# Orca0917/TransformerTTS

Hardware: AMD Instinct MI355X
Metric: mel frames/sec teacher-forced step, LJSpeech-shape batch, 1/2/4/8 MI355X (higher is better)
Workload: dtype f32; 1 GPU; BASELINE configs[2] (batch 64, 1 GPU; per-GPU shard of configs[3]): training step (no-grad fwd + fwd + loss + bwd + clip + Adam), batch 64/GPU x 870 frames x 100 phonemes (dense), base config d_model 256, 3+3 layers, dropout on, fp32; global_batch=64, parallelism=dp1, batch_stream=one resident batch, accumulate=1, process_group=none, grad_allreduce=none (1 GPU), alignments_written=True, dma_gemms=True, layernorm_images=False, head_images=True, fused_cross_kv=True, wgrad_groups=True, twin_encoder=True, twin_postnet=True

## Files before the change

include/ttts_hip.h:

```cpp
#ifndef TTTS_HIP_H
#define TTTS_HIP_H

#include <stddef.h>
#include <stdint.h>

#ifdef __cplusplus
extern "C" {
#endif

#define TTTS_OK 0
#define TTTS_ERR_INVALID (-1)
#define TTTS_ERR_LAUNCH (-2)

#define TTTS_AMAX_SLOTS 1024

#define TTTS_ACT_NONE 0
#define TTTS_ACT_RELU 1
#define TTTS_ACT_TANH 2

typedef struct ttts_step_state {
    uint64_t seed;
    float lr;
    float p_tf;
    int64_t step;
// ... 261 lines not shown
                      const int64_t* frames, const uint8_t* mask, int64_t ld_mask, int B, int Tmax, int Pmax, float* mean,
                      int32_t* counts, void* stream);
int ttts_length_regulate_frames(void);
int ttts_length_regulate_fwd(const float* x, int64_t ld_row, int64_t ld_batch, const int64_t* durations, const int64_t* phoneme_lens,
                             int B, int Pmax, int Tmax, int D, float* y, int64_t* mel_lens, int32_t* index, void* stream);
int ttts_length_regulate_bwd(const float* dy, const int64_t* durations, const int64_t* phoneme_lens, int B, int Pmax, int Tmax, int D,
                             float* dx, int accumulate, void* stream);
int ttts_durations_from_log(const float* log_d, const int64_t* phoneme_lens, int B, int Pmax, float alpha, int64_t min_duration,
                            int64_t* durations, void* stream);
int ttts_variance_embed_fwd(const float* x, int64_t ld_row, int64_t ld_batch, const float* pitch, const float* energy,
                            const float* pitch_bins, int n_pitch, const float* energy_bins, int n_energy, const float* pitch_table,
                            const float* energy_table, const int64_t* phoneme_lens, int B, int Pmax, int D, float* y,
                            int64_t* pitch_ids, int64_t* energy_ids, void* stream);
int ttts_variance_loss_fwd(const float* log_d_pred, const int64_t* durations, const float* pitch_pred, const float* pitch_target,
                           const float* energy_pred, const float* energy_target, const int64_t* phoneme_lens, int B, int Pmax, float w_d,
                           float w_p, float w_e, float* out, void* stream);
int ttts_variance_loss_bwd(const float* log_d_pred, const int64_t* durations, const float* pitch_pred, const float* pitch_target,
                           const float* energy_pred, const float* energy_target, const int64_t* phoneme_lens, int B, int Pmax, float w_d,
                           float w_p, float w_e, const float* gout, float* d_log_d, float* d_pitch, float* d_energy, void* stream);
int ttts_heads_pad_w(const float* src, int64_t ld_src, float* dst, int64_t rows, int H, int head_dim, int width, void* stream);
int ttts_heads_unpad_w(const float* src, float* dst, int64_t ld_dst, int64_t rows, int H, int head_dim, int width, void* stream);
int ttts_attention_fwd_img(const void* q, const void* k, const void* v, const float* q_inv, const float* k_inv,
                           const float* v_inv, float* o, float* lse, float* attn, const int64_t* key_lens, int B, int H, int Tq,
                           int Tk, int ldq, int ldk, int ldv, int ldo, int causal, float q_scale, float drop_p, uint64_t seed,
                           const uint64_t* step_seed, const float* v_amax, float* o_amax_out, float* rowstat_out, int64_t q_inv_rows, int64_t k_inv_rows, int64_t stat_plane,
                           void* stream);
int ttts_attention_bwd_img(const void* q, const void* k, const void* v, const float* q_inv, const float* k_inv,
                           const float* v_inv, const float* o, const float* d_o, const float* rowstat, float* delta, float* dq,
                           float* dk, float* dv, const int64_t* key_lens, int B, int H, int Tq, int Tk, int ldq, int ldk, int ldv,
                           int ldo, int lddq, int lddk, int lddv, int causal, float q_scale, float drop_p, uint64_t seed,
                           const uint64_t* step_seed, const float* do_amax, float* dq_amax_out, float* dkv_amax_out,
                           float* dkv_partials , int q_splits ,
                           int64_t q_inv_rows, int64_t k_inv_rows, int64_t stat_plane, void* stream);

int ttts_embedding_fwd(const int64_t* ids, const float* table, float* out, int64_t n, int vocab, int d,
                       float* out_amax_out , void* stream);
int ttts_embedding_bwd(const int64_t* ids, const float* dout, float* dtable, int64_t n, int vocab, int d, int accumulate,
                       void* stream);
int ttts_posenc_fwd(const float* x, const float* pe, const float* alpha, float* y, int B, int T, int d, float drop_p,
                    uint64_t seed, const uint64_t* step_seed, float* y_amax_out , void* stream);
size_t ttts_posenc_bwd_workspace_bytes(void);
int ttts_posenc_bwd(const float* dy, const float* pe, float* dx, float* dalpha, float* ws, size_t ws_bytes, int B, int T,
                    int d, float drop_p, uint64_t seed, const uint64_t* step_seed, int accumulate, void* stream);
int ttts_relu_dropout_bwd(const float* dy, const float* out, float* dx, int64_t n, float drop_p, float* dx_amax_out,
                          void* stream);
int ttts_dropout_bwd(const float* dy, float* dx, int64_t n, float drop_p, uint64_t seed, const uint64_t* step_seed,
                     float* dx_amax_out, void* stream);
int ttts_zero(void* p, size_t nbytes, void* stream);
int ttts_add(const float* x, const float* y, float* z, int64_t n, void* stream);
int ttts_add3(const float* x, const float* y, const float* w, float* z, int64_t n, void* stream);
int ttts_collate_melspec(const float* ragged, const int64_t* frame_offsets, float* out, int B, int Tmax, int n_mels,
                         void* stream);
int ttts_collate_phoneme(const int64_t* ragged, const int64_t* offsets, int64_t* out, int B, int Pmax, void* stream);

int ttts_rowdot_fwd(const float* x, const float* w, const float* b, float* y, int64_t M, int d, void* stream);
size_t ttts_rowdot_bwd_workspace_bytes(int d);
int ttts_rowdot_bwd(const float* dy, const float* x, const float* w, float* dx_accum, float* dw, float* db, float* ws,
                    size_t ws_bytes, int64_t M, int d, int accumulate, ttts_reduce_queue* queue, void* stream);

size_t ttts_loss_workspace_bytes(void);
int ttts_loss_fwd(const float* pred, const float* post, const float* stop, const float* mel, const int64_t* lens,
                  float* out4, float* ws, size_t ws_bytes, int B, int T, int C, float pos_weight, void* stream);
int ttts_loss_bwd(const float* pred, const float* post, const float* stop, const float* mel, const int64_t* lens,
                  const float* ws, const float* g_total, const float* g_pred_mel, const float* g_post_mel, const float* g_stop,
                  float* dpred, float* dpost, float* dstop, int B, int T, int C, float pos_weight, void* stream);
int ttts_sched_sampling_mix(const float* pred, const float* mel, const float* u, const int64_t* lens, float* out, int B,
// ... 53 lines not shown
```

transformertts_amd/_lib.py:

```python
from __future__ import annotations

import ctypes
import os
from ctypes import c_char_p, c_float, c_int, c_int64, c_size_t, c_uint64, c_void_p

import torch

_HERE = os.path.dirname(os.path.abspath(__file__))
LIB_PATH = os.environ.get("TTTS_LIB", os.path.join(_HERE, "libttts_hip.so"))

P, I, L, F, U, Z = c_void_p, c_int, c_int64, c_float, c_uint64, c_size_t

SIGNATURES = {
    "ttts_last_error": (c_char_p, []),
    "ttts_abi_version": (I, []),
    "ttts_linear_fwd": (I, [P, P, P, P, P, L, I, I, I, F, U, P, I, I, P]),
    "ttts_linear_bwd_data": (I, [P, P, P, P, L, I, I, P, F, P]),
    "ttts_wgrad_workspace_bytes": (Z, [L, I, I, I]),
    "ttts_linear_bwd_weight": (I, [P, P, P, P, P, Z, L, I, I, I, I, I, P, P]),
    "ttts_split_bytes": (Z, [L, L]),
    "ttts_split_image_bytes": (Z, [L, L, I, I, I]),
    "ttts_gemm_tile_choice": (I, [L, I, I, I]),
    "ttts_weight_split": (I, [P, P, I, I, I, I, I, P]),
    "ttts_weight_split_units": (L, [L, L, I, I]),
# ... 19 lines not shown
    "ttts_linear_bwd_data_x6": (I, [P, P, P, P, L, I, I, P, F, P]),
    "ttts_conv1d_fwd_x6": (I, [P, P, P, P, I, I, I, I, I, P]),
    "ttts_conv1d_bwd_data_x6": (I, [P, P, P, I, I, I, I, I, P]),
    "ttts_linear_bwd_weight_x6": (I, [P, P, P, P, P, Z, L, I, I, I, I, I, P, P]),
    "ttts_conv1d_bwd_weight_x6": (I, [P, P, P, P, P, Z, I, I, I, I, I, I, P, P]),
    "ttts_linear_bwd_weight_h3": (I, [P, P, P, P, P, Z, L, I, I, I, I, I, P, P, P, P]),
    "ttts_conv1d_bwd_weight_h3": (I, [P, P, P, P, P, Z, I, I, I, I, I, I, P, P, P, P]),
    "ttts_linear_bwd_weight_h3_parts": (I, [P, P, P, P, I, P, Z, L, I, I, I, P, P, P, P]),
    "ttts_wgrad_group_ok": (I, [L, I, I, I]),
    "ttts_wgrad_group": (I, [I, P, P, P, P, P, P, P, P, P, P, P, P, I, P, P, P, P]),
    "ttts_conv1d_pack_bytes": (Z, [I, I, I]),
    "ttts_conv1d_pack_weight": (I, [P, P, P, I, I, I, P]),
    "ttts_conv1d_fwd": (I, [P, P, P, P, I, I, I, I, I, P]),
    "ttts_conv1d_bwd_data": (I, [P, P, P, I, I, I, I, I, P]),
    "ttts_conv1d_bwd_weight": (I, [P, P, P, P, P, Z, I, I, I, I, I, I, P, P]),
    "ttts_bn_workspace_bytes": (Z, [L, I]),
    "ttts_bn_train_stats": (I, [P, P, P, P, P, P, P, Z, L, I, F, F, P]),
    "ttts_bn_eval_stats": (I, [P, P, P, P, I, F, P]),
    "ttts_bn_apply_fwd": (I, [P, P, P, P, P, P, L, I, I, F, U, P, P, P]),
    "ttts_bn_bwd": (I, [P, P, P, P, P, P, P, P, P, P, Z, L, I, I, F, U, P, I, P, I, P]),
    "ttts_layernorm_fwd": (I, [P, P, P, P, P, P, L, I, F, P, P, P, P]),
    "ttts_layernorm_bwd_workspace_bytes": (Z, [I]),
    "ttts_layernorm_bwd": (I, [P, P, P, P, P, P, P, P, P, Z, L, I, I, P, P, P, P]),
    "ttts_layernorm_bwd_drop": (I, [P, P, P, P, P, P, P, P, P, Z, L, I, I, P, F, U, P, P, P, P, P, P]),
    "ttts_attention_fwd": (I, [P, P, P, P, P, P, P, I, I, I, I, I, I, I, I, I, F, F, U, P, P]),
    "ttts_attention_fwd_x6": (I, [P, P, P, P, P, P, P, I, I, I, I, I, I, I, I, I, F, F, U, P, P]),
    "ttts_attention_fwd_h3": (I, [P, P, P, P, P, P, P, I, I, I, I, I, I, I, I, I, F, F, U, P, P, P, P, P, P, P]),
    "ttts_attention_bwd": (I, [P, P, P, P, P, P, P, P, P, P, P, I, I, I, I, I, I, I, I, I, I, I, I, F, F, U, P, P]),
    "ttts_attention_bwd_x6": (I, [P, P, P, P, P, P, P, P, P, P, P, I, I, I, I, I, I, I, I, I, I, I, I, F, F, U, P, P]),
    "ttts_attention_bwd_h3": (I, [P, P, P, P, P, P, P, P, P, P, P, I, I, I, I, I, I, I, I, I, I, I, I, F, F, U, P, P, P, P, P, P, P, P, P]),
    "ttts_attention_fwd_img": (I, [P, P, P, P, P, P, P, P, P, P, I, I, I, I, I, I, I, I, I, F, F, U, P, P, P, P, L, L, L, P]),
    "ttts_attention_bwd_img": (I, [P, P, P, P, P, P, P, P, P, P, P, P, P, P, I, I, I, I, I, I, I, I, I, I, I, I, F, F, U, P, P, P, P,
                                   P, I, L, L, L, P]),
    "ttts_attention_fwd_wide": (I, [P, P, P, P, P, P, P, I, I, I, I, I, I, I, I, I, F, F, U, P, P]),
    "ttts_attention_bwd_wide": (I, [P, P, P, P, P, P, P, P, P, P, P, I, I, I, I, I, I, I, I, I, I, I, I, F, F, U, P, P]),
    "ttts_attention_fwd_wide_masked": (I, [P, P, P, P, P, P, P, I, I, I, I, I, I, I, I, I, F, F, U, P, P, L, L, L, P, L, P]),
    "ttts_attention_bwd_wide_masked": (I, [P, P, P, P, P, P, P, P, P, P, P, I, I, I, I, I, I, I, I, I, I, I, I, F, F, U, P, P, L, L, L,
                                           P, L, P]),
    "ttts_attention_bwd_wide_dattn": (I, [P, P, P, P, P, P, P, P, P, P, P, I, I, I, I, I, I, I, I, I, I, I, I, F, F, U, P, P, L, L, L,
                                          P, L, P, P, L, L, L, P]),
    "ttts_guided_attention_fwd": (I, [P, P, P, U, F, I, I, I, I, P, I, I, I, P, P]),
    "ttts_guided_attention_bwd": (I, [P, P, P, U, F, I, I, I, I, I, I, P, P]),
    "ttts_alignment_rowstats": (I, [P, L, L, L, P, P, I, I, I, I, I, I, P, P, P, P]),
    "ttts_alignment_select": (I, [P, P, P, I, I, I, I, I, I, P, P, P]),
    "ttts_alignment_durations_argmax": (I, [P, P, P, P, I, I, I, I, I, P, P, P]),
    "ttts_alignment_mas_workspace_bytes": (Z, [I, I, I]),
    "ttts_alignment_mas": (I, [P, I, L, L, L, P, P, P, I, I, I, I, P, Z, P, P, P]),
    "ttts_dtw_workspace_bytes": (Z, [I, I, I]),
    "ttts_dtw": (I, [P, L, L, P, P, L, L, P, I, I, I, I, I, P, Z, P, P, P, P, P, P]),
    "ttts_audio_tables_bytes": (Z, [I, I, I]),
    "ttts_audio_tables_check": (I, [P, Z, I, I, I, I]),
    "ttts_logmel": (I, [P, L, P, I, I, I, I, I, I, P, F, P, P, P, I, P]),
    "ttts_logmel_stats": (I, [P, P, I, I, I, P, P]),
    "ttts_vocoder_pinv_check": (I, [P, Z, I, I]),
    "ttts_mel_to_magnitude": (I, [P, L, L, P, I, I, I, I, I, P, P, F, P, P, P]),
    "ttts_istft": (I, [P, P, I, I, I, I, P, P, P, P]),
    "ttts_stft_project": (I, [P, L, P, P, I, I, I, I, P, P, P, F, P, P, P]),
    "ttts_resample_table_bytes": (Z, [I, I]),
    "ttts_resample_table_check": (I, [P, Z, I, I, I]),
    "ttts_resample_tile": (I, []),
    "ttts_resample": (I, [P, L, P, I, I, I, I, I, P, P, L, P, P]),
    "ttts_pitch_lags": (I, []),
    "ttts_pitch_frames": (I, [I, I, I, I, I]),
    "ttts_pitch_block": (I, [I, I, I, I, I]),
    "ttts_pitch_energy": (I, [P, L, P, I, I, I, I, I, I, I, I, I, F, F, P, P, P, P, P, P, P]),
    "ttts_segment_mean": (I, [P, L, P, P, P, P, L, I, I, I, P, P, P]),
# ... 84 lines not shown
```

transformertts_amd/csrc/attention_img.hip:

```cpp
#include "attention_common.h"

namespace ttts {

struct AttnImgArgs {
    const void* q; const void* k; const void* v;
    const float* q_inv; const float* k_inv; const float* v_inv;
    long q_rows, k_rows;
    long stat_plane;
    float* o; float* lse; float* attn;
    const float* dout; float* delta; float* dq; float* dk; float* dv;
    const int64_t* key_lens;
    int B, H, Tq, Tk;
    int ldq, ldk, ldv, ldo, lddq, lddk, lddv;
    float qscale;
    float drop_scale; uint32_t thr; uint64_t seed; const uint64_t* step_seed;
    const float* v_amax;
    const float* do_amax;
    float* amax_dq; float* amax_dkv;
    float* dkv_part; long part_stride;
    int ldp;
    float* o_amax;
    float* rowstat;
};

// ... 1075 lines not shown
        const float fv = inv_g / H3A_P * a.drop_scale;
        float mx = 0.f;
#pragma unroll
        for (int r = 0; r < 16; ++r) {
            dk[0][r] *= fk; dk[1][r] *= fk; dv[0][r] *= fv; dv[1][r] *= fv;
            mx = fmaxf(fmaxf(mx, fmaxf(fabsf(dk[0][r]), fabsf(dk[1][r]))), fmaxf(fabsf(dv[0][r]), fabsf(dv[1][r])));
        }
        if (a.amax_dkv != nullptr && gridDim.z == 1) amax_publish(kg < a.Tk ? mx : 0.f, a.amax_dkv, blockIdx.y * gridDim.x + blockIdx.x);
    }
    if (gridDim.z == 1) {
        wave_store_rows4(dk, scratch4, a.dk + (long)b * a.Tk * a.lddk + h * HD, kw0, a.Tk, a.lddk, lane);
        wave_store_rows4(dv, scratch4, a.dv + (long)b * a.Tk * a.lddv + h * HD, kw0, a.Tk, a.lddv, lane);
    } else {
        float* part = a.dkv_part + (long)blockIdx.z * a.part_stride + (long)b * a.Tk * a.ldp + h * HD;
        wave_store_rows4(dk, scratch4, part, kw0, a.Tk, a.ldp, lane);
        wave_store_rows4(dv, scratch4, part + a.H * HD, kw0, a.Tk, a.ldp, lane);
    }
}

__global__ __launch_bounds__(256) void attn_dkv_reduce_kernel(const float* __restrict__ part, float* __restrict__ out, long n4, int zs,
                                                              long stride, float* __restrict__ amax, int cols4, long out_ld) {
    float mx = 0.f;
    for (long i = (long)blockIdx.x * blockDim.x + threadIdx.x; i < n4; i += (long)gridDim.x * blockDim.x) {
        float4 acc = reinterpret_cast<const float4*>(part)[i];
        for (int z = 1; z < zs; ++z) {
            const float4 v = reinterpret_cast<const float4*>(part + (long)z * stride)[i];
            acc.x += v.x; acc.y += v.y; acc.z += v.z; acc.w += v.w;
        }
        const long row = i / cols4;
        *reinterpret_cast<float4*>(out + row * out_ld + (i - row * cols4) * 4) = acc;
        mx = fmaxf(fmaxf(mx, fmaxf(fabsf(acc.x), fabsf(acc.y))), fmaxf(fabsf(acc.z), fabsf(acc.w)));
    }
    if (amax != nullptr) amax_publish(mx, amax, blockIdx.x * 4 + (threadIdx.x >> 6));
}

#ifndef TTTS_AIMG_KT
#define TTTS_AIMG_KT 32
#endif

static int check_img_spans(const char* name, int Tq, int Tk, int ldq, int ldk, int ldv) {
    TTTS_REQUIRE((uint64_t)Tq * ldq * 4 < (1ull << 32) && (uint64_t)Tk * ldk * 4 < (1ull << 32) && (uint64_t)Tk * ldv * 4 < (1ull << 32),
                 "%s: one utterance's operand exceeds 4 GiB", name);
    return TTTS_OK;
}
static int fill_img_planes(const char* name, AttnImgArgs& a, int B, int H, int Tq, int Tk, int64_t q_inv_rows, int64_t k_inv_rows,
                           int64_t stat_plane) {
    TTTS_REQUIRE((q_inv_rows == 0 || q_inv_rows >= (int64_t)B * Tq) && (k_inv_rows == 0 || k_inv_rows >= (int64_t)B * Tk) &&
                 (stat_plane == 0 || stat_plane >= (int64_t)B * H * Tq), "%s: plane strides smaller than the batch", name);
    a.q_rows = q_inv_rows ? q_inv_rows : (long)B * Tq; a.k_rows = k_inv_rows ? k_inv_rows : (long)B * Tk;
    a.stat_plane = stat_plane ? stat_plane : (long)B * H * Tq;
    return TTTS_OK;
}

}

using namespace ttts;

#ifdef TTTS_AIMG_STAMPS
extern "C" int ttts_dbg_aimg_read_stamps(unsigned long long* host, size_t n) {
    return (int)hipMemcpyFromSymbol(host, HIP_SYMBOL(ttts::ttts_aimg_stamps), n * sizeof(unsigned long long));
}
#endif

extern "C" int ttts_attention_fwd_img(const void* q, const void* k, const void* v, const float* q_inv, const float* k_inv,
                                      const float* v_inv, float* o, float* lse, float* attn, const int64_t* key_lens, int B, int H,
                                      int Tq, int Tk, int ldq, int ldk, int ldv, int ldo, int causal, float q_scale, float drop_p,
                                      uint64_t seed, const uint64_t* step_seed, const float* v_amax, float* o_amax_out,
                                      float* rowstat_out, int64_t q_inv_rows, int64_t k_inv_rows, int64_t stat_plane, void* stream) {
    TTTS_REQUIRE(q && k && v && q_inv && k_inv && v_inv && o && key_lens && v_amax, "attention_fwd_img: null pointer");
    int rc = attn_check("attention_fwd_img", HD, B, H, Tq, Tk, ldq, ldk, ldv, ldo, causal, drop_p);
    if (!rc) rc = check_img_spans("attention_fwd_img", Tq, Tk, ldq, ldk, ldv);
    if (rc) return rc;
    TTTS_REQUIRE(!(causal && attn), "attention_fwd_img: weights output is only for non-causal (cross) attention");
    TTTS_REQUIRE((((uintptr_t)q | (uintptr_t)k | (uintptr_t)v | (uintptr_t)o | (uintptr_t)v_amax) & 15) == 0,
                 "attention_fwd_img: q/k/v/o/v_amax must be 16-byte aligned");
    AttnImgArgs a = {};
    attn_fill(a, key_lens, B, H, Tq, Tk, ldq, ldk, ldv, ldo, q_scale, drop_p, seed, step_seed);
    rc = fill_img_planes("attention_fwd_img", a, B, H, Tq, Tk, q_inv_rows, k_inv_rows, stat_plane);
    if (rc) return rc;
    a.q = q; a.k = k; a.v = v; a.q_inv = q_inv; a.k_inv = k_inv; a.v_inv = v_inv;
    a.o = o; a.lse = lse; a.attn = attn;
    a.v_amax = v_amax; a.o_amax = o_amax_out; a.rowstat = rowstat_out;
    dim3 grid(B * H, cdiv(Tq, QB), 1);
    if (causal)
        hipLaunchKernelGGL((attn_fwd_img_kernel<true, false, TTTS_AIMG_KT>), grid, dim3(256), 0, (hipStream_t)stream, a);
    else if (!attn)
        hipLaunchKernelGGL((attn_fwd_img_kernel<false, false, TTTS_AIMG_KT>), grid, dim3(256), 0, (hipStream_t)stream, a);
    else if (Tk <= 128)
        hipLaunchKernelGGL(attn_fwd_img_maps_kernel, grid, dim3(256), 0, (hipStream_t)stream, a);
    else
        hipLaunchKernelGGL((attn_fwd_img_kernel<false, true, 64>), grid, dim3(256), 0, (hipStream_t)stream, a);
    TTTS_LAUNCH_CHECK("attn_fwd_img_kernel");
    return TTTS_OK;
}

extern "C" int ttts_attention_bwd_img(const void* q, const void* k, const void* v, const float* q_inv, const float* k_inv,
                                      const float* v_inv, const float* o, const float* d_o, const float* rowstat, float* delta,
                                      float* dq, float* dk, float* dv, const int64_t* key_lens, int B, int H, int Tq, int Tk, int ldq,
                                      int ldk, int ldv, int ldo, int lddq, int lddk, int lddv, int causal, float q_scale,
                                      float drop_p, uint64_t seed, const uint64_t* step_seed, const float* do_amax,
                                      float* dq_amax_out, float* dkv_amax_out, float* dkv_partials, int q_splits,
                                      int64_t q_inv_rows, int64_t k_inv_rows, int64_t stat_plane, void* stream_) {
    hipStream_t stream = (hipStream_t)stream_;
    TTTS_REQUIRE(q && k && v && q_inv && k_inv && v_inv && o && d_o && rowstat && delta && dq && dk && dv && key_lens && do_amax,
                 "attention_bwd_img: null pointer");
    int rc = attn_check("attention_bwd_img", HD, B, H, Tq, Tk, ldq, ldk, ldv, ldo, causal, drop_p);
    if (!rc) rc = check_img_spans("attention_bwd_img", Tq, Tk, ldq, ldk, ldv);
    if (!rc) rc = attn_check_grad_strides("attention_bwd_img", HD, H, lddq, lddk, lddv);
    if (rc) return rc;
    TTTS_REQUIRE((((uintptr_t)q | (uintptr_t)k | (uintptr_t)v | (uintptr_t)o | (uintptr_t)d_o | (uintptr_t)do_amax) & 15) == 0,
                 "attention_bwd_img: q/k/v/o/d_o/do_amax must be 16-byte aligned");
    TTTS_REQUIRE((uint64_t)Tq * ldo * 4 < (1ull << 32), "attention_bwd_img: one utterance's d_o exceeds 4 GiB");
    AttnImgArgs a = {};
    attn_fill(a, key_lens, B, H, Tq, Tk, ldq, ldk, ldv, ldo, q_scale, drop_p, seed, step_seed);
    rc = fill_img_planes("attention_bwd_img", a, B, H, Tq, Tk, q_inv_rows, k_inv_rows, stat_plane);
    if (rc) return rc;
    a.q = q; a.k = k; a.v = v; a.q_inv = q_inv; a.k_inv = k_inv; a.v_inv = v_inv;
    a.o = const_cast<float*>(o); a.dout = d_o; a.delta = delta; a.dq = dq; a.dk = dk; a.dv = dv;
    a.lddq = lddq; a.lddk = lddk; a.lddv = lddv;
    a.do_amax = do_amax; a.amax_dq = dq_amax_out; a.amax_dkv = dkv_amax_out;
    a.rowstat = const_cast<float*>(rowstat);
    TTTS_REQUIRE(q_splits >= 1 && q_splits <= 16, "attention_bwd_img: q_splits out of 1..16");
    if (q_splits > 1) {
        TTTS_REQUIRE(dkv_partials && dv == dk + H * HD && lddk >= 2 * H * HD && lddv == lddk,
                     "attention_bwd_img: query splits need a workspace and a (dk | dv) gradient whose rows hold dk then dv");
        a.ldp = 2 * H * HD;
        a.dkv_part = dkv_partials; a.part_stride = (long)B * Tk * a.ldp;
    }
    rc = ATTN_LAUNCH_BWD(attn_bwd_dq_img_kernel, 0, attn_bwd_dkv_img_kernel, 0, causal, "attention_bwd_img", "attn_bwd_dq_img_kernel",
                         "attn_bwd_dkv_img_kernel", a, q_splits, stream);
    if (rc) return rc;
    if (q_splits > 1) {
        const long n4 = a.part_stride / 4;
        const long blocks = (n4 + 255) / 256;
        hipLaunchKernelGGL(attn_dkv_reduce_kernel, dim3((unsigned)(blocks < 2048 ? blocks : 2048)), dim3(256), 0, stream, dkv_partials, dk, n4,
                           q_splits, a.part_stride, dkv_amax_out, a.ldp / 4, (long)lddk);
        TTTS_LAUNCH_CHECK("attn_dkv_reduce_kernel");
    }
    return TTTS_OK;
}
```

transformertts_amd/ops.py:

```python
from __future__ import annotations

import os
import weakref
from ctypes import c_void_p
from typing import NamedTuple, Optional

import torch

from . import _lib

ACT_NONE, ACT_RELU, ACT_TANH = 0, 1, 2
AMAX_SLOTS = 1024


def _p(t: Optional[torch.Tensor]):
    return None if t is None else c_void_p(t.data_ptr())


_raw_stream = getattr(torch._C, "_cuda_getCurrentRawStream", None)


def _stream():
    if _raw_stream is not None:
        return c_void_p(_raw_stream(torch.cuda.current_device()))
# ... 863 lines not shown
_relu_observer = None
_drop_observer = None


def _saw_drop(kind: str, seed: int, p: float, shape, half=None) -> None:
    if _drop_observer is not None and float(p) > 0.0:
        _drop_observer(kind, int(seed), float(p), tuple(int(v) for v in shape), half)


class _ReluToken:
    __slots__ = ("scale", "premasked")

    def __init__(self, scale: float):
        self.scale, self.premasked = scale, False


class _DropToken:
    __slots__ = ("p", "seed", "ss", "dx", "dacc", "amax", "image")

    def __init__(self, p: float, seed: int, ss):
        self.p, self.seed, self.ss = p, seed, ss
        self.dx = self.dacc = self.amax = self.image = None


class SkipToken:
    __slots__ = ("grad",)

    def __init__(self):
        self.grad = None


HEAD_IMAGES = True
FUSED_CROSS_KV = True


class HeadImage:
    __slots__ = ("cells", "row_inv", "sec_amax", "sec_cols", "col0", "slab", "index")

    def __init__(self, cells, row_inv, sec_amax, sec_cols: int, col0: int = 0, slab=None, index: int = 0):
        self.cells, self.row_inv, self.sec_amax, self.sec_cols, self.col0, self.slab, self.index = \
            cells, row_inv, sec_amax, int(sec_cols), int(col0), slab, int(index)

    @property
    def shape(self):
        return self.cells.shape

    @property
    def device(self):
        return self.cells.device

    @property
    def ld(self) -> int:
        return self.cells.stride(-2)

    def inv_of(self, col: int):
        rows = self.row_inv.shape[1]
        return _off(self.row_inv, ((self.col0 + col) // 64) * rows)

    def amax_of(self, col: int) -> torch.Tensor:
        return self.sec_amax[(self.col0 + col) // self.sec_cols]

    def __repr__(self):
        return f"HeadImage(shape={tuple(self.shape)}, ld={self.ld}, col0={self.col0})"


def head_image_ok(x: torch.Tensor, w: torch.Tensor, n_head: int, sections: int) -> bool:
# ... 659 lines not shown


def _dattn_operand(g: torch.Tensor, Tk: int) -> torch.Tensor:
    if g.dtype != torch.float32:
        g = g.to(torch.float32)
    return g if _dattn_in_place(g, Tk) else pad_mask_rows(g)


def _dattn_args(g4: torch.Tensor, Tk: int):
    return _rows_args(g4, Tk)


def _off(t: torch.Tensor, col: int):
    return c_void_p(t.data_ptr() + 4 * col)


def _img_operand(cells: torch.Tensor, himg: "HeadImage", col: int):
    return _off(cells, col), cells.stride(1), himg.inv_of(col), himg.row_inv.shape[1]


def _attn_img_fwd(q, k, v, o, stat, attn, lens, B, H, Tq, Tk, causal, drop_p, seed, v_am, o_am) -> None:
    lib = _lib.load()
    (qp, ldq, qi, q_rows), (kp, ldk, ki, k_rows), (vp, ldv, vi, _) = q, k, v
    _lib.check(lib.ttts_attention_fwd_img(qp, kp, vp, qi, ki, vi, _p(o), _p(stat[0]), _p(attn), _p(lens), B, H, Tq, Tk, ldq, ldk,
                                          ldv, o.shape[-1], 1 if causal else 0, 0.125, float(drop_p), seed, _ss(), _p(v_am),
                                          _p(o_am), _p(stat[1:]), q_rows, k_rows, stat.stride(0), _stream()),
               "ttts_attention_fwd_img")


def _attn_img_bwd(q, k, v, o, do, stat, delta, dq, dk, dv, lens, B, H, Tq, Tk, causal, drop_p, seed, ss, dq_am, dkv_am,
                  partials=None, q_splits: int = 1) -> None:
    lib = _lib.load()
    (qp, ldq, qi, q_rows), (kp, ldk, ki, k_rows), (vp, ldv, vi, _) = q, k, v
    _lib.check(lib.ttts_attention_bwd_img(qp, kp, vp, qi, ki, vi, _p(o), _p(do), _p(stat[1:]), _p(delta), dq[0], dk[0], dv[0],
                                          _p(lens), B, H, Tq, Tk, ldq, ldk, ldv, o.shape[-1], dq[1], dk[1], dv[1],
                                          1 if causal else 0, 0.125, drop_p, seed, ss, _p(_amax(do)), _p(dq_am), _p(dkv_am),
                                          _p(partials), q_splits, q_rows, k_rows, stat.stride(0), _stream()),
               "ttts_attention_bwd_img")


def _head_width(d: int, n_head: int) -> int:
    if n_head <= 0 or d % n_head != 0:
        raise ValueError(f"attention: d_model {d} is not divisible by {n_head} heads")
    return d // n_head


def masked_attention(q, k, v, lens, n_head: int, causal: bool, drop_p: float, dead=None, add_mask=None):
    B, Tq, d = q.shape
    Tk = k.shape[1]
    hd = _head_width(d, n_head)
    qh = q.reshape(B, Tq, n_head, hd).transpose(1, 2)
    kh = k.reshape(B, Tk, n_head, hd).transpose(1, 2)
    vh = v.reshape(B, Tk, n_head, hd).transpose(1, 2)
    s = torch.matmul(qh * hd ** -0.5, kh.transpose(-1, -2))
    key = torch.arange(Tk, device=q.device)
    if dead is None:
        dead = key[None, :] >= lens.to(q.device)[:, None]
    big = torch.finfo(torch.float32).min
    if add_mask is not None:
        s = s + add_mask
    s = s.masked_fill(dead[:, None, None, :], big)
    if causal:
        s = s.masked_fill((key[None, :] > torch.arange(Tq, device=q.device)[:, None])[None, None], big)
    p = torch.softmax(s, dim=-1) * (s > 0.5 * big).any(dim=-1, keepdim=True).to(s.dtype)
    if drop_p > 0:
        p = torch.nn.functional.dropout(p, drop_p, True)
    o = torch.matmul(p, vh).transpose(1, 2).reshape(B, Tq, d)
    return o, p


def _pad_heads(src: torch.Tensor, col0: int, ld: int, rows: int, H: int, hd: int, width: int = 64) -> torch.Tensor:
# ... 591 lines not shown
```

Before: 4.266 million mel frames/s.

## Fuse attention backward dq and dk/dv into one-pass kernel for short keys

Adds a one-pass attention backward kernel for the head-image path. Each workgroup keeps all keys (up to 128) resident in registers and streams query tiles, computing dk/dv and dq in the same sweep instead of running separate dq and dkv kernels. It is used for non-causal attention with Tk <= 128, which fits the cross-attention over 100 phonemes. This removes a second pass over Q, dO and the recomputed softmax, at the cost of heavier LDS use (two workgroups per CU) and new dq accumulation and scaling logic.

```diff
diff --git a/include/ttts_hip.h b/include/ttts_hip.h
--- a/include/ttts_hip.h
+++ b/include/ttts_hip.h
@@ -317,6 +317,13 @@
                            const uint64_t* step_seed, const float* do_amax, float* dq_amax_out, float* dkv_amax_out,
                            float* dkv_partials , int q_splits ,
                            int64_t q_inv_rows, int64_t k_inv_rows, int64_t stat_plane, void* stream);
+int ttts_attention_bwd_img_onepass(const void* q, const void* k, const void* v, const float* q_inv, const float* k_inv,
+                                   const float* v_inv, const float* o, const float* d_o, const float* rowstat, float* delta,
+                                   float* dq, float* dk, float* dv, const int64_t* key_lens, int B, int H, int Tq, int Tk, int ldq,
+                                   int ldk, int ldv, int ldo, int lddq, int lddk, int lddv, int causal, float q_scale,
+                                   float drop_p, uint64_t seed, const uint64_t* step_seed, const float* do_amax,
+                                   float* dq_amax_out, float* dkv_amax_out, float* dkv_partials, int q_splits,
+                                   int64_t q_inv_rows, int64_t k_inv_rows, int64_t stat_plane, void* stream);
 
 int ttts_embedding_fwd(const int64_t* ids, const float* table, float* out, int64_t n, int vocab, int d,
                        float* out_amax_out , void* stream);
diff --git a/transformertts_amd/_lib.py b/transformertts_amd/_lib.py
--- a/transformertts_amd/_lib.py
+++ b/transformertts_amd/_lib.py
@@ -75,6 +75,8 @@
     "ttts_attention_fwd_img": (I, [P, P, P, P, P, P, P, P, P, P, I, I, I, I, I, I, I, I, I, F, F, U, P, P, P, P, L, L, L, P]),
     "ttts_attention_bwd_img": (I, [P, P, P, P, P, P, P, P, P, P, P, P, P, P, I, I, I, I, I, I, I, I, I, I, I, I, F, F, U, P, P, P, P,
                                    P, I, L, L, L, P]),
+    "ttts_attention_bwd_img_onepass": (I, [P, P, P, P, P, P, P, P, P, P, P, P, P, P, I, I, I, I, I, I, I, I, I, I, I, I, F, F, U, P, P,
+                                           P, P, P, I, L, L, L, P]),
     "ttts_attention_fwd_wide": (I, [P, P, P, P, P, P, P, I, I, I, I, I, I, I, I, I, F, F, U, P, P]),
     "ttts_attention_bwd_wide": (I, [P, P, P, P, P, P, P, P, P, P, P, I, I, I, I, I, I, I, I, I, I, I, I, F, F, U, P, P]),
     "ttts_attention_fwd_wide_masked": (I, [P, P, P, P, P, P, P, I, I, I, I, I, I, I, I, I, F, F, U, P, P, L, L, L, P, L, P]),
diff --git a/transformertts_amd/csrc/attention_img.hip b/transformertts_amd/csrc/attention_img.hip
--- a/transformertts_amd/csrc/attention_img.hip
+++ b/transformertts_amd/csrc/attention_img.hip
@@ -1131,6 +1131,365 @@
         mx = fmaxf(fmaxf(mx, fmaxf(fabsf(acc.x), fabsf(acc.y))), fmaxf(fabsf(acc.z), fabsf(acc.w)));
     }
     if (amax != nullptr) amax_publish(mx, amax, blockIdx.x * 4 + (threadIdx.x >> 6));
+}
+
+constexpr int OP_TLD = 36;
+constexpr int OP_PART = 32 * OUT_LD * 4;
+constexpr int OP_LDS = 2 * DKI_STAGE + 4 * OP_PART;
+constexpr int OP_KSTEP = 32 * OP_TLD * 4;
+static_assert(OP_KSTEP >= 2 * 2048 && OP_KSTEP + 2 * 2048 <= OP_PART, "scratch and K'^T staging alias the wave's partial tile");
+static_assert(OUT_BYTES <= 2 * DKI_STAGE, "the epilogue's scratch aliases the stages");
+__global__ __launch_bounds__(256, 2) void attn_bwd_onepass_img_kernel(AttnImgArgs a) {
+    const uint64_t seed_eff = site_seed(a.seed, a.step_seed);
+    const uint32_t thr16 = a.thr << 16;
+    extern __shared__ __attribute__((aligned(16))) char xs[];
+    __shared__ float red4[4];
+
+    const int tid = threadIdx.x, lane = tid & 63;
+    const int wave = __builtin_amdgcn_readfirstlane(tid >> 6);
+    const int l31 = lane & 31, half = lane >> 5;
+    const int h = blockIdx.x % a.H, b = blockIdx.x / a.H;
+    const int kw0 = wave * 32;
+    const int kg = kw0 + l31;
+    const uint32_t key_mult = attn_drop_mult((uint32_t)kg);
+    float* scratch4 = reinterpret_cast<float*>(xs) + wave * 32 * OUT_LD;
+    float* part = reinterpret_cast<float*>(xs + 2 * DKI_STAGE);
+    float* tile = part + wave * (OP_PART / 4);
+
+    const int klen = attn_klen(a.key_lens, b, a.Tk);
+    const int nlive = (klen + 31) >> 5;
+    const long arow = ((long)(b * a.H + h) * a.Tq);
+
+    float s_g, inv_g;
+    img_tensor_scale(a.do_amax, lane, wave, red4, s_g, inv_g);
+
+    const int fsw = isw(l31);
+    const uint32_t r_off0 = (uint32_t)(l31 * 128 + ((half ^ fsw) << 4));
+    auto r_off = [&](int st) { return r_off0 ^ (uint32_t)(st << 5); };
+    const int q4 = (lane & 15) >> 2, pc = lane & 3, g16 = (lane >> 4) & 1;
+    const uint32_t t_off0 = (uint32_t)((4 * half + q4) * 128 + (((2 * g16 + (pc >> 1)) ^ isw(4 * half + q4)) << 4) + (pc & 1) * 8);
+    auto t_off = [&](int i2, int sc) { return (t_off0 ^ (uint32_t)(i2 * 64 + sc * 32)) + (uint32_t)(sc * 1024); };
+    const int ld_r = lane >> 3;
+
+    const int krow = kg < a.Tk ? kg : a.Tk - 1;
+    f16x8v kf[4][2], vf[4][2];
+    {
+        const char* kp = reinterpret_cast<const char*>(a.k) + ((long)(b * a.Tk + krow) * a.ldk + h * HD) * 4;
+        const char* vp = reinterpret_cast<const char*>(a.v) + ((long)(b * a.Tk + krow) * a.ldv + h * HD) * 4;
+#pragma unroll
+        for (int s = 0; s < 4; ++s)
+#pragma unroll
+            for (int p = 0; p < 2; ++p) {
+                kf[s][p] = *reinterpret_cast<const f16x8v*>(kp + p * 128 + (2 * s + half) * 16);
+                vf[s][p] = *reinterpret_cast<const f16x8v*>(vp + p * 128 + (2 * s + half) * 16);
+            }
+    }
+    const float kinv = a.k_inv[(long)h * a.k_rows + (long)b * a.Tk + krow];
+    const float vinv = a.v_inv[(long)h * a.k_rows + (long)b * a.Tk + krow];
+
+    f32x16 dk[2], dv[2];
+#pragma unroll
+    for (int r = 0; r < 16; ++r) { dk[0][r] = 0.f; dk[1][r] = 0.f; dv[0][r] = 0.f; dv[1][r] = 0.f; }
+
+    const float dp_unscale = inv_g * vinv * a.drop_scale;
+    float sds = 0.f;
+    float mxq = 0.f;
+    const int nqs_all = (a.Tq + DKI_QS - 1) / DKI_QS;
+    const int per_z = (nqs_all + (int)gridDim.z - 1) / (int)gridDim.z;
+    const int nqs = min(nqs_all, ((int)blockIdx.z + 1) * per_z);
+    const int qs_begin = min((int)blockIdx.z * per_z, nqs);
+
+    const u32x4a rsQ = make_rsrc(reinterpret_cast<const char*>(a.q) + ((long)b * a.Tq * a.ldq + h * HD) * 4, (uint32_t)a.Tq * (uint32_t)a.ldq * 4u);
+    const u32x4a rsG = make_rsrc(a.dout + (long)b * a.Tq * a.ldo + h * HD, (uint32_t)a.Tq * (uint32_t)a.ldo * 4u);
+    const long plane = a.stat_plane;
+    const uint32_t lds0 = lds_addr_a(xs);
+    const uint32_t ld_cq = (uint32_t)((lane & 7) ^ isw(8 * (wave & 1) + ld_r)) * 16u;
+    float4 o_lo, o_hi;
+    float st_f;
+    auto fetch_row = [&](int qt0) {
+        int row = qt0 + 8 * wave + ld_r;
+        row = row < a.Tq ? row : a.Tq - 1;
+        const float* op = a.o + ((long)b * a.Tq + row) * a.ldo + h * HD + (lane & 7) * 8;
+        o_lo = *reinterpret_cast<const float4*>(op);
+        o_hi = *reinterpret_cast<const float4*>(op + 4);
+        st_f = a.rowstat[(long)min(lane & 7, 4) * plane + arow + row];
+    };
+    auto issue = [&](int qt0, int stage) {
+        const uint32_t dst = lds0 + (uint32_t)stage * DKI_STAGE;
+        int row = qt0 + 8 * wave + ld_r;
+        row = row < a.Tq ? row : a.Tq - 1;
+        const uint32_t qo = (uint32_t)row * (uint32_t)(a.ldq * 4) + ld_cq;
+        const uint32_t go = (uint32_t)row * (uint32_t)(a.ldo * 4) + (uint32_t)(lane & 7) * 16u;
+        const uint32_t piece = (uint32_t)(8 * wave) * 128u;
+#pragma unroll
+        for (int p = 0; p < 2; ++p) {
+            dma16a(rsQ, qo, (uint32_t)p * 128u, __builtin_amdgcn_readfirstlane(dst + (uint32_t)p * DKI_PLANE + piece));
+            dma16a(rsG, go, (uint32_t)p * 128u, __builtin_amdgcn_readfirstlane(dst + (uint32_t)(2 + p) * DKI_PLANE + piece));
+        }
+    };
+    auto convert = [&](int qt0, int stage) {
+        char* st_ = xs + stage * DKI_STAGE;
+        const int row = 8 * wave + ld_r, c = lane & 7;
+        const char* src = st_ + (2 + (c >> 2)) * DKI_PLANE + row * 128 + (c & 3) * 32;
+        const float4 x0 = *reinterpret_cast<const float4*>(src), x1 = *reinterpret_cast<const float4*>(src + 16);
+        asm volatile("s_waitcnt lgkmcnt(0)" ::: "memory");
+        __builtin_amdgcn_wave_barrier();
+        u32x4a hi, lo;
+        uint32_t hh, ll;
+        split2_pair_h(f32x2{x0.x, x0.y} * s_g, hh, ll); hi.x = hh; lo.x = ll;
+        split2_pair_h(f32x2{x0.z, x0.w} * s_g, hh, ll); hi.y = hh; lo.y = ll;
+        split2_pair_h(f32x2{x1.x, x1.y} * s_g, hh, ll); hi.z = hh; lo.z = ll;
+        split2_pair_h(f32x2{x1.z, x1.w} * s_g, hh, ll); hi.w = hh; lo.w = ll;
+        const int off = row * 128 + ((c ^ isw(row)) << 4);
+        *reinterpret_cast<u32x4a*>(st_ + 2 * DKI_PLANE + off) = hi;
+        *reinterpret_cast<u32x4a*>(st_ + 3 * DKI_PLANE + off) = lo;
+        float d = x0.x * o_lo.x;
+        d = __builtin_fmaf(x0.y, o_lo.y, d); d = __builtin_fmaf(x0.z, o_lo.z, d); d = __builtin_fmaf(x0.w, o_lo.w, d);
+        d = __builtin_fmaf(x1.x, o_hi.x, d); d = __builtin_fmaf(x1.y, o_hi.y, d); d = __builtin_fmaf(x1.z, o_hi.z, d);
+        d = __builtin_fmaf(x1.w, o_hi.w, d);
+        d += __shfl_xor(d, 1, 64);
+        d += __shfl_xor(d, 2, 64);
+        d += __shfl_xor(d, 4, 64);
+        const bool saturated = __shfl(st_f, (lane & ~7) | 2, 64) != 0.f;
+        float* stat = reinterpret_cast<float*>(st_ + 4 * DKI_PLANE);
+        if (c < 5) {
+            const float v = c == 2 ? (saturated ? 0.f : 1.f) : (c == 4 && saturated) ? 0.f : st_f;
+            stat[(c == 2 ? 288 : 64 * c) + row] = v;
+        }
+        if (c == 0) {
+            d = saturated ? -0.f : d;
+            stat[128 + row] = d;
+            if (qt0 + row < a.Tq) a.delta[arow + qt0 + row] = d;
+        }
+    };
+
+#pragma unroll
+    for (int st = 0; st < 4; ++st)
+#pragma unroll
+        for (int p = 0; p < 2; ++p) asm volatile("" : "+v"(kf[st][p]), "+v"(vf[st][p]));
+    if (qs_begin < nqs) {
+        issue(qs_begin * DKI_QS, qs_begin & 1);
+        fetch_row(qs_begin * DKI_QS);
+        asm volatile("s_waitcnt vmcnt(0)" ::: "memory");
+        convert(qs_begin * DKI_QS, qs_begin & 1);
+    }
+    asm volatile("s_waitcnt lgkmcnt(0)\n\ts_barrier" ::: "memory");
+
+    const bool skip = kw0 >= klen;
+    for (int qs = qs_begin; qs < nqs; ++qs) {
+        const int qt0 = qs * DKI_QS;
+        if (qs + 1 < nqs) issue(qt0 + DKI_QS, (qs + 1) & 1);
+        const char* st_ = xs + (qs & 1) * DKI_STAGE;
+        if (!skip) {
+            f32x16 s, dp;
+#pragma unroll
+            for (int r = 0; r < 16; ++r) { s[r] = 0.f; dp[r] = 0.f; }
+#pragma unroll
+            for (int st = 0; st < 4; ++st) {
+                f16x8v qfr[2];
+#pragma unroll
+                for (int p = 0; p < 2; ++p) qfr[p] = *reinterpret_cast<const f16x8v*>(st_ + p * DKI_PLANE + r_off(st));
+                s = __builtin_amdgcn_mfma_f32_32x32x16_f16(qfr[0], kf[st][1], s, 0, 0, 0);
+                s = __builtin_amdgcn_mfma_f32_32x32x16_f16(qfr[1], kf[st][0], s, 0, 0, 0);
+                s = __builtin_amdgcn_mfma_f32_32x32x16_f16(qfr[0], kf[st][0], s, 0, 0, 0);
+            }
+            const bool full = (kw0 + 32 <= klen) && (qt0 + DKI_QS <= a.Tq);
+            const float* stat = reinterpret_cast<const float*>(st_ + 4 * DKI_PLANE);
+            float pd[16];
+#pragma unroll
+            for (int g4 = 0; g4 < 4; ++g4) {
+                const float4 m4 = *reinterpret_cast<const float4*>(stat + 8 * g4 + 4 * half);
+                const float4 l4 = *reinterpret_cast<const float4*>(stat + 64 + 8 * g4 + 4 * half);
+                const float4 e4 = *reinterpret_cast<const float4*>(stat + 192 + 8 * g4 + 4 * half);
+                const float mq4[4] = {m4.x, m4.y, m4.z, m4.w}, l24[4] = {l4.x, l4.y, l4.z, l4.w}, c24[4] = {e4.x, e4.y, e4.z, e4.w};
+#pragma unroll
+                for (int e = 0; e < 4; ++e) {
+                    const int r = 4 * g4 + e;
+                    pd[r] = fast_exp2(__builtin_fmaf(s[r] * kinv, c24[e], -mq4[e]) - l24[e]);
+                }
+            }
+            if (!full) {
+#pragma unroll
+                for (int r = 0; r < 16; ++r) {
+                    const int q_g = qt0 + acc_row(r, half);
+                    pd[r] = (kg < klen && q_g < a.Tq) ? pd[r] : 0.f;
+                }
+            }
+#pragma unroll
+            for (int st = 0; st < 4; ++st) {
+                f16x8v gfr[2];
+#pragma unroll
+                for (int p = 0; p < 2; ++p) gfr[p] = *reinterpret_cast<const f16x8v*>(st_ + (2 + p) * DKI_PLANE + r_off(st));
+                mfma_h3(dp, gfr, vf[st]);
+            }
+            float ds[16];
+#pragma unroll
+            for (int r = 0; r < 16; r += 4) {
+                uint32_t hq[4];
+                {
+                    const int rr = r + (lane & 3);
+                    const uint32_t mine = attn_quad_hash(seed_eff, (uint32_t)(arow + qt0 + acc_row(rr, half)), (uint32_t)kg >> 2);
+                    hq[0] = (uint32_t)__builtin_amdgcn_mov_dpp((int)mine, 0x00, 0xF, 0xF, true);
+                    hq[1] = (uint32_t)__builtin_amdgcn_mov_dpp((int)mine, 0x55, 0xF, 0xF, true);
+                    hq[2] = (uint32_t)__builtin_amdgcn_mov_dpp((int)mine, 0xAA, 0xF, 0xF, true);
+                    hq[3] = (uint32_t)__builtin_amdgcn_mov_dpp((int)mine, 0xFF, 0xF, 0xF, true);
+                }
+                const float4 d4 = *reinterpret_cast<const float4*>(stat + 128 + 2 * r + 4 * half);
+                const float4 f4 = *reinterpret_cast<const float4*>(stat + 256 + 2 * r + 4 * half);
+                const float4 v4 = *reinterpret_cast<const float4*>(stat + 288 + 2 * r + 4 * half);
+                const float dl4[4] = {d4.x, d4.y, d4.z, d4.w}, cq4[4] = {f4.x, f4.y, f4.z, f4.w}, lv4[4] = {v4.x, v4.y, v4.z, v4.w};
+#pragma unroll
+                for (int e = 0; e < 4; ++e) {
+                    float g = dp[r + e] * dp_unscale;
+                    float pk = pd[r + e];
+                    {
+                        const bool keep = attn_keep_word(hq[e], key_mult, thr16);
+                        g = keep ? g : 0.f;
+                        pk = keep ? pk : 0.f;
+                    }
+                    const float t = pd[r + e] * (g - dl4[e]);
+                    ds[r + e] = t * cq4[e];
+                    tile[acc_row(r + e, half) * OP_TLD + l31] = t * (kinv * lv4[e]);
+                    pd[r + e] = pk;
+                }
+            }
+            attn_h3_track_scale(ds, sds, dk);
+#pragma unroll
+            for (int t2 = 0; t2 < 2; ++t2) {
+                float x[8];
+                f16x8v f[2];
+#pragma unroll
+                for (int e = 0; e < 8; ++e) x[e] = pd[8 * t2 + e];
+                split_frag8_h3(x, H3A_P, f[0], f[1]);
+#pragma unroll
+                for (int i2 = 0; i2 < 2; ++i2) {
+                    f16x8v af[2];
+#pragma unroll
+                    for (int pl = 0; pl < 2; ++pl) {
+                        const char* gb = st_ + (2 + pl) * DKI_PLANE + t2 * 2048;
+                        af[pl] = join_tr(lds_tr4(gb + t_off(i2, 0)), lds_tr4(gb + t_off(i2, 1)));
+                    }
+                    mfma_h3(dv[i2], af, f);
+                }
+#pragma unroll
+                for (int e = 0; e < 8; ++e) x[e] = ds[8 * t2 + e];
+                split_frag8_h3(x, sds, f[0], f[1]);
+#pragma unroll
+                for (int i2 = 0; i2 < 2; ++i2) {
+                    f16x8v af[2];
+#pragma unroll
+                    for (int pl = 0; pl < 2; ++pl) {
+                        const char* qb = st_ + pl * DKI_PLANE + t2 * 2048;
+                        af[pl] = join_tr(lds_tr4(qb + t_off(i2, 0)), lds_tr4(qb + t_off(i2, 1)));
+                    }
+                    mfma_h3(dk[i2], af, f);
+                }
+            }
+        }
+        if (qs + 1 < nqs) fetch_row(qt0 + DKI_QS);
+        if (!skip) {
+            wave_lds_sync();
+            float xq[16];
+#pragma unroll
+            for (int g4 = 0; g4 < 4; ++g4) {
+                const float4 t4 = *reinterpret_cast<const float4*>(tile + l31 * OP_TLD + 8 * g4 + 4 * half);
+                xq[4 * g4] = t4.x; xq[4 * g4 + 1] = t4.y; xq[4 * g4 + 2] = t4.z; xq[4 * g4 + 3] = t4.w;
+            }
+            wave_lds_sync();
+            {
+                char* kt = reinterpret_cast<char*>(tile) + (l31 >> 4) * OP_KSTEP + (l31 & 15) * 128;
+#pragma unroll
+                for (int pl = 0; pl < 2; ++pl)
+#pragma unroll
+                    for (int st = 0; st < 4; ++st)
+                        *reinterpret_cast<f16x8v*>(kt + pl * 2048 + (((2 * st + half) ^ fsw) << 4)) = kf[st][pl];
+            }
+            wave_lds_sync();
+            float m = 0.f;
+#pragma unroll
+            for (int r = 0; r < 16; ++r) m = fmaxf(m, fabsf(xq[r]));
+            m = fmaxf(m, __shfl_xor(m, 32, 64));
+            const uint32_t ex = (__float_as_uint(m) >> 23) & 0xffu;
+            const bool scaled = ex >= 24u && ex < 255u;
+            const float sq = scaled ? __uint_as_float((265u - ex) << 23) : 0.f;
+            const float sq_inv = scaled ? __uint_as_float((ex - 11u) << 23) : 0.f;
+            f32x16 dqp[2];
+#pragma unroll
+            for (int r = 0; r < 16; ++r) { dqp[0][r] = 0.f; dqp[1][r] = 0.f; }
+#pragma unroll
+            for (int t2 = 0; t2 < 2; ++t2) {
+                float x[8];
+                f16x8v f[2];
+#pragma unroll
+                for (int e = 0; e < 8; ++e) x[e] = xq[8 * t2 + e];
+                split_frag8_h3(x, sq, f[0], f[1]);
+#pragma unroll
+                for (int i2 = 0; i2 < 2; ++i2) {
+                    f16x8v ktf[2];
+#pragma unroll
+                    for (int pl = 0; pl < 2; ++pl) {
+                        const char* kb = reinterpret_cast<const char*>(tile) + t2 * OP_KSTEP + pl * 2048;
+                        ktf[pl] = join_tr(lds_tr4(kb + t_off(i2, 0)), lds_tr4(kb + t_off(i2, 1)));
+                    }
+                    mfma_h3(dqp[i2], ktf, f);
+                }
+            }
+            wave_lds_sync();
+#pragma unroll
+            for (int i2 = 0; i2 < 2; ++i2)
+#pragma unroll
+                for (int g4 = 0; g4 < 4; ++g4)
+                    *reinterpret_cast<float4*>(tile + l31 * OUT_LD + i2 * 32 + 8 * g4 + 4 * half) =
+                        make_float4(dqp[i2][4 * g4] * sq_inv, dqp[i2][4 * g4 + 1] * sq_inv, dqp[i2][4 * g4 + 2] * sq_inv,
+                                    dqp[i2][4 * g4 + 3] * sq_inv);
+        }
+        asm volatile("s_waitcnt lgkmcnt(0)\n\ts_barrier" ::: "memory");
+        asm volatile("s_waitcnt vmcnt(0)" ::: "memory");
+        if (qs + 1 < nqs) convert(qt0 + DKI_QS, (qs + 1) & 1);
+        {
+            const int row = 8 * wave + ld_r, c4 = (lane & 7) * 4;
+            const float* p0 = part + row * OUT_LD + c4;
+            float4 s0 = make_float4(0.f, 0.f, 0.f, 0.f), s1 = s0;
+#pragma unroll
+            for (int w2 = 0; w2 < 4; ++w2)
+                if (w2 < nlive) {
+                    const float4 u0 = *reinterpret_cast<const float4*>(p0 + w2 * (OP_PART / 4));
+                    const float4 u1 = *reinterpret_cast<const float4*>(p0 + w2 * (OP_PART / 4) + 32);
+                    s0.x += u0.x; s0.y += u0.y; s0.z += u0.z; s0.w += u0.w;
+                    s1.x += u1.x; s1.y += u1.y; s1.z += u1.z; s1.w += u1.w;
+                }
+            s0.x *= a.qscale; s0.y *= a.qscale; s0.z *= a.qscale; s0.w *= a.qscale;
+            s1.x *= a.qscale; s1.y *= a.qscale; s1.z *= a.qscale; s1.w *= a.qscale;
+            if (qt0 + row < a.Tq) {
+                float* dst = a.dq + ((long)b * a.Tq + qt0 + row) * a.lddq + h * HD + c4;
+                *reinterpret_cast<float4*>(dst) = s0;
+                *reinterpret_cast<float4*>(dst + 32) = s1;
+                mxq = fmaxf(mxq, fmaxf(fmaxf(fmaxf(fabsf(s0.x), fabsf(s0.y)), fmaxf(fabsf(s0.z), fabsf(s0.w))),
+                                       fmaxf(fmaxf(fabsf(s1.x), fabsf(s1.y)), fmaxf(fabsf(s1.z), fabsf(s1.w)))));
+            }
+        }
+        asm volatile("s_waitcnt lgkmcnt(0)\n\ts_barrier" ::: "memory");
+    }
+    if (a.amax_dq != nullptr) amax_publish(mxq, a.amax_dq, blockIdx.z * gridDim.x + blockIdx.x);
+    {
+        const float fk = (sds > 0.f) ? 1.f / sds : 0.f;
+        const float fv = inv_g / H3A_P * a.drop_scale;
+        float mx = 0.f;
+#pragma unroll
+        for (int r = 0; r < 16; ++r) {
+            dk[0][r] *= fk; dk[1][r] *= fk; dv[0][r] *= fv; dv[1][r] *= fv;
+            mx = fmaxf(fmaxf(mx, fmaxf(fabsf(dk[0][r]), fabsf(dk[1][r]))), fmaxf(fabsf(dv[0][r]), fabsf(dv[1][r])));
+        }
+        if (a.amax_dkv != nullptr && gridDim.z == 1) amax_publish(kg < a.Tk ? mx : 0.f, a.amax_dkv, blockIdx.x);
+    }
+    if (gridDim.z == 1) {
+        wave_store_rows4(dk, scratch4, a.dk + (long)b * a.Tk * a.lddk + h * HD, kw0, a.Tk, a.lddk, lane);
+        wave_store_rows4(dv, scratch4, a.dv + (long)b * a.Tk * a.lddv + h * HD, kw0, a.Tk, a.lddv, lane);
+    } else {
+        float* ps = a.dkv_part + (long)blockIdx.z * a.part_stride + (long)b * a.Tk * a.ldp + h * HD;
+        wave_store_rows4(dk, scratch4, ps, kw0, a.Tk, a.ldp, lane);
+        wave_store_rows4(dv, scratch4, ps + a.H * HD, kw0, a.Tk, a.ldp, lane);
+    }
 }
 
 #ifndef TTTS_AIMG_KT
@@ -1193,6 +1552,69 @@
     return TTTS_OK;
 }
 
+static int attention_bwd_img_entry(const char* name, bool onepass, const void* q, const void* k, const void* v, const float* q_inv, const float* k_inv,
+                                   const float* v_inv, const float* o, const float* d_o, const float* rowstat, float* delta,
+                                   float* dq, float* dk, float* dv, const int64_t* key_lens, int B, int H, int Tq, int Tk, int ldq,
+                                   int ldk, int ldv, int ldo, int lddq, int lddk, int lddv, int causal, float q_scale,
+                                   float drop_p, uint64_t seed, const uint64_t* step_seed, const float* do_amax,
+                                   float* dq_amax_out, float* dkv_amax_out, float* dkv_partials, int q_splits,
+                                   int64_t q_inv_rows, int64_t k_inv_rows, int64_t stat_plane, void* stream_) {
+    hipStream_t stream = (hipStream_t)stream_;
+    TTTS_REQUIRE(q && k && v && q_inv && k_inv && v_inv && o && d_o && rowstat && delta && dq && dk && dv && key_lens && do_amax,
+                 "%s: null pointer", name);
+    int rc = attn_check(name, HD, B, H, Tq, Tk, ldq, ldk, ldv, ldo, causal, drop_p);
+    if (!rc) rc = check_img_spans(name, Tq, Tk, ldq, ldk, ldv);
+    if (!rc) rc = attn_check_grad_strides(name, HD, H, lddq, lddk, lddv);
+    if (rc) return rc;
+    TTTS_REQUIRE(!onepass || (!causal && Tk <= QB), "%s: the one-pass form is not causal and holds every key in one %d-key block (causal %d, Tk %d)",
+                 name, QB, causal, Tk);
+    TTTS_REQUIRE((((uintptr_t)q | (uintptr_t)k | (uintptr_t)v | (uintptr_t)o | (uintptr_t)d_o | (uintptr_t)do_amax) & 15) == 0,
+                 "%s: q/k/v/o/d_o/do_amax must be 16-byte aligned", name);
+    TTTS_REQUIRE((uint64_t)Tq * ldo * 4 < (1ull << 32), "%s: one utterance's d_o exceeds 4 GiB", name);
+    AttnImgArgs a = {};
+    attn_fill(a, key_lens, B, H, Tq, Tk, ldq, ldk, ldv, ldo, q_scale, drop_p, seed, step_seed);
+    rc = fill_img_planes(name, a, B, H, Tq, Tk, q_inv_rows, k_inv_rows, stat_plane);
+    if (rc) return rc;
+    a.q = q; a.k = k; a.v = v; a.q_inv = q_inv; a.k_inv = k_inv; a.v_inv = v_inv;
+    a.o = const_cast<float*>(o); a.dout = d_o; a.delta = delta; a.dq = dq; a.dk = dk; a.dv = dv;
+    a.lddq = lddq; a.lddk = lddk; a.lddv = lddv;
+    a.do_amax = do_amax; a.amax_dq = dq_amax_out; a.amax_dkv = dkv_amax_out;
+    a.rowstat = const_cast<float*>(rowstat);
+    TTTS_REQUIRE(q_splits >= 1 && q_splits <= 16, "%s: q_splits out of 1..16", name);
+    if (q_splits > 1) {
+        TTTS_REQUIRE(dkv_partials && dv == dk + H * HD && lddk >= 2 * H * HD && lddv == lddk,
+                     "%s: query splits need a workspace and a (dk | dv) gradient whose rows hold dk then dv", name);
+        a.ldp = 2 * H * HD;
+        a.dkv_part = dkv_partials; a.part_stride = (long)B * Tk * a.ldp;
+    }
+    if (onepass) {
+        static bool configured = false;
+        if (!configured) {
+            const hipError_t e = hipFuncSetAttribute(reinterpret_cast<const void*>(attn_bwd_onepass_img_kernel),
+                                                     hipFuncAttributeMaxDynamicSharedMemorySize, OP_LDS);
+            if (e != hipSuccess) {
+                set_error("%s: cannot reserve %d bytes of LDS: %s", name, OP_LDS, hipGetErrorString(e));
+                return TTTS_ERR_LAUNCH;
+            }
+            configured = true;
+        }
+        hipLaunchKernelGGL(attn_bwd_onepass_img_kernel, dim3(B * H, 1, q_splits), dim3(256), OP_LDS, stream, a);
+        TTTS_LAUNCH_CHECK("attn_bwd_onepass_img_kernel");
+    } else {
+        rc = ATTN_LAUNCH_BWD(attn_bwd_dq_img_kernel, 0, attn_bwd_dkv_img_kernel, 0, causal, name, "attn_bwd_dq_img_kernel",
+                             "attn_bwd_dkv_img_kernel", a, q_splits, stream);
+        if (rc) return rc;
+    }
+    if (q_splits > 1) {
+        const long n4 = a.part_stride / 4;
+        const long blocks = (n4 + 255) / 256;
+        hipLaunchKernelGGL(attn_dkv_reduce_kernel, dim3((unsigned)(blocks < 2048 ? blocks : 2048)), dim3(256), 0, stream, dkv_partials, dk, n4,
+                           q_splits, a.part_stride, dkv_amax_out, a.ldp / 4, (long)lddk);
+        TTTS_LAUNCH_CHECK("attn_dkv_reduce_kernel");
+    }
+    return TTTS_OK;
+}
+
 extern "C" int ttts_attention_bwd_img(const void* q, const void* k, const void* v, const float* q_inv, const float* k_inv,
                                       const float* v_inv, const float* o, const float* d_o, const float* rowstat, float* delta,
                                       float* dq, float* dk, float* dv, const int64_t* key_lens, int B, int H, int Tq, int Tk, int ldq,
@@ -1200,41 +1622,19 @@
                                       float drop_p, uint64_t seed, const uint64_t* step_seed, const float* do_amax,
                                       float* dq_amax_out, float* dkv_amax_out, float* dkv_partials, int q_splits,
                                       int64_t q_inv_rows, int64_t k_inv_rows, int64_t stat_plane, void* stream_) {
-    hipStream_t stream = (hipStream_t)stream_;
-    TTTS_REQUIRE(q && k && v && q_inv && k_inv && v_inv && o && d_o && rowstat && delta && dq && dk && dv && key_lens && do_amax,
-                 "attention_bwd_img: null pointer");
-    int rc = attn_check("attention_bwd_img", HD, B, H, Tq, Tk, ldq, ldk, ldv, ldo, causal, drop_p);
-    if (!rc) rc = check_img_spans("attention_bwd_img", Tq, Tk, ldq, ldk, ldv);
-    if (!rc) rc = attn_check_grad_strides("attention_bwd_img", HD, H, lddq, lddk, lddv);
-    if (rc) return rc;
-    TTTS_REQUIRE((((uintptr_t)q | (uintptr_t)k | (uintptr_t)v | (uintptr_t)o | (uintptr_t)d_o | (uintptr_t)do_amax) & 15) == 0,
-                 "attention_bwd_img: q/k/v/o/d_o/do_amax must be 16-byte aligned");
-    TTTS_REQUIRE((uint64_t)Tq * ldo * 4 < (1ull << 32), "attention_bwd_img: one utterance's d_o exceeds 4 GiB");
-    AttnImgArgs a = {};
-    attn_fill(a, key_lens, B, H, Tq, Tk, ldq, ldk, ldv, ldo, q_scale, drop_p, seed, step_seed);
-    rc = fill_img_planes("attention_bwd_img", a, B, H, Tq, Tk, q_inv_rows, k_inv_rows, stat_plane);
-    if (rc) return rc;
-    a.q = q; a.k = k; a.v = v; a.q_inv = q_inv; a.k_inv = k_inv; a.v_inv = v_inv;
-    a.o = const_cast<float*>(o); a.dout = d_o; a.delta = delta; a.dq = dq; a.dk = dk; a.dv = dv;
-    a.lddq = lddq; a.lddk = lddk; a.lddv = lddv;
-    a.do_amax = do_amax; a.amax_dq = dq_amax_out; a.amax_dkv = dkv_amax_out;
-    a.rowstat = const_cast<float*>(rowstat);
-    TTTS_REQUIRE(q_splits >= 1 && q_splits <= 16, "attention_bwd_img: q_splits out of 1..16");
-    if (q_splits > 1) {
-        TTTS_REQUIRE(dkv_partials && dv == dk + H * HD && lddk >= 2 * H * HD && lddv == lddk,
-                     "attention_bwd_img: query splits need a workspace and a (dk | dv) gradient whose rows hold dk then dv");
-        a.ldp = 2 * H * HD;
-        a.dkv_part = dkv_partials; a.part_stride = (long)B * Tk * a.ldp;
-    }
-    rc = ATTN_LAUNCH_BWD(attn_bwd_dq_img_kernel, 0, attn_bwd_dkv_img_kernel, 0, causal, "attention_bwd_img", "attn_bwd_dq_img_kernel",
-                         "attn_bwd_dkv_img_kernel", a, q_splits, stream);
-    if (rc) return rc;
-    if (q_splits > 1) {
-        const long n4 = a.part_stride / 4;
-        const long blocks = (n4 + 255) / 256;
-        hipLaunchKernelGGL(attn_dkv_reduce_kernel, dim3((unsigned)(blocks < 2048 ? blocks : 2048)), dim3(256), 0, stream, dkv_partials, dk, n4,
-                           q_splits, a.part_stride, dkv_amax_out, a.ldp / 4, (long)lddk);
-        TTTS_LAUNCH_CHECK("attn_dkv_reduce_kernel");
-    }
-    return TTTS_OK;
-}
+    return attention_bwd_img_entry("attention_bwd_img", false, q, k, v, q_inv, k_inv, v_inv, o, d_o, rowstat, delta, dq, dk, dv, key_lens, B, H, Tq, Tk, ldq, ldk, ldv,
+                                   ldo, lddq, lddk, lddv, causal, q_scale, drop_p, seed, step_seed, do_amax, dq_amax_out, dkv_amax_out,
+                                   dkv_partials, q_splits, q_inv_rows, k_inv_rows, stat_plane, stream_);
+}
+
+extern "C" int ttts_attention_bwd_img_onepass(const void* q, const void* k, const void* v, const float* q_inv, const float* k_inv,
+                                              const float* v_inv, const float* o, const float* d_o, const float* rowstat, float* delta,
+                                              float* dq, float* dk, float* dv, const int64_t* key_lens, int B, int H, int Tq, int Tk, int ldq,
+                                              int ldk, int ldv, int ldo, int lddq, int lddk, int lddv, int causal, float q_scale,
+                                              float drop_p, uint64_t seed, const uint64_t* step_seed, const float* do_amax,
+                                              float* dq_amax_out, float* dkv_amax_out, float* dkv_partials, int q_splits,
+                                              int64_t q_inv_rows, int64_t k_inv_rows, int64_t stat_plane, void* stream_) {
+    return attention_bwd_img_entry("attention_bwd_img_onepass", true, q, k, v, q_inv, k_inv, v_inv, o, d_o, rowstat, delta, dq, dk, dv, key_lens, B, H, Tq, Tk, ldq, ldk, ldv,
+                                   ldo, lddq, lddk, lddv, causal, q_scale, drop_p, seed, step_seed, do_amax, dq_amax_out, dkv_amax_out,
+                                   dkv_partials, q_splits, q_inv_rows, k_inv_rows, stat_plane, stream_);
+}
diff --git a/transformertts_amd/ops.py b/transformertts_amd/ops.py
--- a/transformertts_amd/ops.py
+++ b/transformertts_amd/ops.py
@@ -919,6 +919,7 @@
 
 HEAD_IMAGES = True
 FUSED_CROSS_KV = True
+ONEPASS_ATTN_BWD = True
 
 
 class HeadImage:
@@ -1644,11 +1645,11 @@
                   partials=None, q_splits: int = 1) -> None:
     lib = _lib.load()
     (qp, ldq, qi, q_rows), (kp, ldk, ki, k_rows), (vp, ldv, vi, _) = q, k, v
-    _lib.check(lib.ttts_attention_bwd_img(qp, kp, vp, qi, ki, vi, _p(o), _p(do), _p(stat[1:]), _p(delta), dq[0], dk[0], dv[0],
-                                          _p(lens), B, H, Tq, Tk, ldq, ldk, ldv, o.shape[-1], dq[1], dk[1], dv[1],
-                                          1 if causal else 0, 0.125, drop_p, seed, ss, _p(_amax(do)), _p(dq_am), _p(dkv_am),
-                                          _p(partials), q_splits, q_rows, k_rows, stat.stride(0), _stream()),
-               "ttts_attention_bwd_img")
+    name = "ttts_attention_bwd_img_onepass" if ONEPASS_ATTN_BWD and not causal and Tk <= 128 else "ttts_attention_bwd_img"
+    _lib.check(getattr(lib, name)(qp, kp, vp, qi, ki, vi, _p(o), _p(do), _p(stat[1:]), _p(delta), dq[0], dk[0], dv[0],
+                                  _p(lens), B, H, Tq, Tk, ldq, ldk, ldv, o.shape[-1], dq[1], dk[1], dv[1],
+                                  1 if causal else 0, 0.125, drop_p, seed, ss, _p(_amax(do)), _p(dq_am), _p(dkv_am),
+                                  _p(partials), q_splits, q_rows, k_rows, stat.stride(0), _stream()), name)
 
 
 def _head_width(d: int, n_head: int) -> int:
```

Result: no change. 4.308 million mel frames/s, median of 6 (+1.0%).
